# roymor1/OptimalStrategiesAgainstGenerativeAttacks

Measured on AMD Instinct MI355X. Metric: GIM episodes/sec (64x64x3, m=1 n=5 k=10), higher is better.
Workload: dtype f32

## Files before the change

### include/gim_hip.h

```cpp
#ifndef GIM_HIP_H
#define GIM_HIP_H

#include <stddef.h>
#include <stdint.h>

#ifdef __cplusplus
extern "C" {
#endif

#define GIM_OK 0
#define GIM_E_BADARG (-1)
#define GIM_E_LAUNCH (-2)

const char* gim_last_error(void);
int gim_version(void);

typedef struct {
    int32_t N, H, W, Cin, Cout, KH, ups;
    float pre_slope;
    int32_t pool, wfold, res_ups;
    int32_t tune_tile, tune_ksplit, tune_wgrad;
    int32_t out_zeroed;
    float post_slope;
    int32_t prec;
} gim_conv_shape;

int gim_conv2d_fold_weights(const float* w, float* f, int Cout, int Cin, int KH, void* stream);
typedef struct {
    const float* w;
    float* f;
    int32_t Cout, Cin, KH, reserved;
} gim_fold_job;
int gim_conv2d_fold_weights_batched(const gim_fold_job* jobs, const int32_t* tab, int n_blocks, void* stream);

int gim_conv2d_fwd(const float* x, const float* w, const float* bias, const float* sigma, const float* residual,
                   float* y, const gim_conv_shape* s, void* stream);

int gim_conv2d_dgrad(const float* dy, const float* w, const float* sigma, const float* mask_x, float* dx,
                     const gim_conv_shape* s, void* stream);

int gim_conv2d_dgrad_res(const float* dy, const float* w, const float* sigma, const float* mask_x, const float* res_half,
                         float res_scale, float* dx, const gim_conv_shape* s, void* stream);

int gim_conv2d_wgrad_slabs(const gim_conv_shape* s);
int gim_conv2d_wgrad(const float* dy, const float* x, float* slabs, float* bias_slabs, int n_slabs, const gim_conv_shape* s,
                     void* stream);

int gim_wgrad_finish(const float* slabs, const float* bias_slabs, int n_slabs, const float* w, const float* sigma,
                     const float* u, const float* v, float* dw, float* db, float* scratch, int Cout, int Cin, int KH,
                     int fold, float* acc_dw, float* acc_db, void* stream);

int gim_spectral_sigma(const float* w, float* u, float* v, float* sigma, float* u_out, float* v_out, float* scratch,
                       int Cout, int Cin, int KH, int training, void* stream);

typedef struct {
    const float* w;
    float* u;
    float* v;
    int64_t off_sigma, off_u, off_v, off_scratch;
    int32_t Cout, Cin, KH, reserved;
} gim_sn_job;
int gim_spectral_sigma_batched(const gim_sn_job* jobs, int n_jobs, const int32_t* tab_cols, int n_col_blocks,
                               const int32_t* tab_rows, int n_row_blocks, float* out_base, int training, void* stream);

int gim_conv2d_transpose_weights(const float* w, float* wt, int Cout, int Cin, int KF, void* stream);
int gim_conv2d_dgrad_t(const float* dy, const float* wt, const float* sigma, const float* mask_x, float* dx,
                       const gim_conv_shape* shape, void* stream);

int gim_conv2d_xfold_weights(const float* w, float* wx, int Cout, int Cin, int KH, int J, void* stream);
int gim_conv2d_dgrad_xfold(const float* dy, const float* wx, const float* sigma, const float* mask_x, float* dx,
                           const gim_conv_shape* shape, int J, void* stream);

int gim_pad_image(const float* x, float* xp, int N, int H, int W, int C, int pad, float slope, void* stream);
int gim_conv2d_pack_rows_weights(const float* w, float* wp, int Cout, int Cin, int KH, void* stream);
int gim_conv2d_fwd_rows(const float* xp, const float* wp, const float* bias, const float* sigma, const float* residual,
                        float* y, const gim_conv_shape* shape, void* stream);
int gim_conv2d_wgrad_rows_acc(const float* dy, const float* xp, float* acc, float* bias_acc, const gim_conv_shape* shape, void* stream);

int gim_conv2d_pack_subpixel_weights(const float* wf, float* wm, int Cout, int Cin, int KH, void* stream);
int gim_depth_to_space2(const float* y4, const float* bias, float* y, int N, int Hs, int Ws, int C, float post_slope, void* stream);

int gim_conv_launch_plan(const gim_conv_shape* shape, int kind, int32_t* out);

int gim_conv2d_wgrad_acc(const float* dy, const float* x, float* acc, float* bias_acc, const gim_conv_shape* shape, void* stream);

typedef struct {
    const float* src;
    const float* bias_src;
    const float* w;
    const float* sigma;
    const float* u;
    const float* v;
    float* tmp;
    float* partial;
    float* grad_w;
    float* grad_b;
    int32_t Cout, Cin, K, fold;
    int32_t n_chunks, exclusive;
} gim_wgrad_job;
int gim_wgrad_finish_batched(const gim_wgrad_job* jobs, int n_jobs, const int32_t* tab, int n_blocks, const int32_t* tab_sn,
                             int n_blocks_sn, void* stream);

int gim_colsum(const float* x, float* out, float* scratch, int64_t rows, int C, void* stream);

int gim_colsum_acc(const float* x, float* out, float* scratch, int64_t rows, int C, void* stream);
int gim_colsum2(const float* a, const float* b, float* out_a, float* out_b, int rows, int C, int accumulate, void* stream);

int gim_norm_fwd(const float* x, const float* scale, const float* shift, const float* residual, float* y, float* stats,
                 int N, int HW, int C, int mode, float eps, void* stream);
int gim_norm_fwd_act(const float* x, const float* scale, const float* shift, const float* residual, float* y, float* stats,
                     int N, int HW, int C, int mode, float eps, float post_slope, void* stream);
int gim_norm_bwd(const float* dy, const float* x, const float* scale, const float* stats, float* dx, float* dscale_nc,
                 float* dshift_nc, int N, int HW, int C, int mode, void* stream);

int gim_avgpool2_fwd(const float* x, float* y, int N, int H, int W, int C, void* stream);
int gim_avgpool2_fwd_act(const float* x, float* y, int N, int H, int W, int C, float in_slope, void* stream);
int gim_add_n(const float* a, const float* b, const float* c, const float* d, float* out, int64_t n, void* stream);
int gim_add_avgpool2_bwd(const float* g, const float* dy_pooled, float* out, int N, int H, int W, int C, void* stream);
int gim_avgpool2_bwd(const float* dy, float* dx, int N, int H, int W, int C, void* stream);
int gim_upsample2x_bwd(const float* dy_up, const float* mask_x, float slope, float* dx, int N, int H, int W, int C, void* stream);

int gim_maxpool_lrelu_fwd(const float* x, float* y, int32_t* idx, int N, int HW, int C, float slope, void* stream);
int gim_maxpool_lrelu_bwd(const float* dy, const float* y, const int32_t* idx, float* dx, int N, int HW, int C, float slope, void* stream);

int gim_attn_prob_fwd(const float* f, const float* g, float* P, int batch, int T, int K, void* stream);

int gim_bgemm(const float* A, const float* B, float* C, int batch, int M, int N, int K,
              int64_t sAb, int64_t sAi, int64_t sAk, int64_t sBb, int64_t sBk, int64_t sBj, void* stream);

typedef struct {
    const float* A;
    const float* B;
    float* C;
    const float* bias;
    int32_t M, N, K, ldc;
    int64_t sAi, sAk, sBk, sBj;
    int32_t flags, reserved;
} gim_gemm_job;
int gim_bgemm_grouped(const gim_gemm_job* jobs, const int32_t* tiles, int n_tiles, void* stream);
int gim_colsum_grouped(const gim_gemm_job* jobs, const int32_t* tiles, int n_tiles, void* stream);

int gim_softmax_dim1_fwd(const float* s, float* p, int B, int R, int Ccols, void* stream);
int gim_softmax_dim1_bwd(const float* dp, const float* p, float* ds, int B, int R, int Ccols, void* stream);

int gim_scale_add_fwd(const float* a, const float* x, const float* gamma, float* y, int64_t n, void* stream);
int gim_scale_add_fwd_act(const float* a, const float* x, const float* gamma, float* y, int64_t n, float post_slope, void* stream);
// ... 73 lines not shown
```

### optimalstrategiesagainstgenerativeattacks_amd/_lib.py

```python
import ctypes
import os
from ctypes import POINTER, c_float, c_int, c_int32, c_int64, c_void_p

_HERE = os.path.dirname(os.path.abspath(__file__))
LIB_PATH = os.environ.get("GIM_LIB_PATH") or os.path.join(_HERE, "csrc", "libgim_hip.so")


class GimConvShape(ctypes.Structure):
    _fields_ = [("N", c_int32), ("H", c_int32), ("W", c_int32), ("Cin", c_int32), ("Cout", c_int32),
                ("KH", c_int32), ("ups", c_int32), ("pre_slope", c_float),
                ("pool", c_int32), ("wfold", c_int32), ("res_ups", c_int32),
                ("tune_tile", c_int32), ("tune_ksplit", c_int32), ("tune_wgrad", c_int32),
                ("out_zeroed", c_int32), ("post_slope", c_float), ("prec", c_int32)]


class GimInferConv(ctypes.Structure):
    _fields_ = [("N", c_int32), ("H", c_int32), ("W", c_int32), ("Cin", c_int32), ("Cout", c_int32),
                ("KH", c_int32), ("stride", c_int32)]


P = c_void_p
SP = POINTER(GimConvShape)


class GimFoldJob(ctypes.Structure):
    _fields_ = [("w", P), ("f", P), ("Cout", c_int32), ("Cin", c_int32), ("KH", c_int32), ("reserved", c_int32)]


class GimSnJob(ctypes.Structure):
    _fields_ = [("w", P), ("u", P), ("v", P), ("off_sigma", c_int64), ("off_u", c_int64), ("off_v", c_int64), ("off_scratch", c_int64),
                ("Cout", c_int32), ("Cin", c_int32), ("KH", c_int32), ("reserved", c_int32)]


class GimWgradJob(ctypes.Structure):
    _fields_ = [("src", P), ("bias_src", P), ("w", P), ("sigma", P), ("u", P), ("v", P), ("tmp", P), ("partial", P),
                ("grad_w", P), ("grad_b", P), ("Cout", c_int32), ("Cin", c_int32), ("K", c_int32), ("fold", c_int32),
                ("n_chunks", c_int32), ("exclusive", c_int32)]


class GimGemmJob(ctypes.Structure):
    _fields_ = [("A", P), ("B", P), ("C", P), ("bias", P), ("M", c_int32), ("N", c_int32), ("K", c_int32), ("ldc", c_int32),
                ("sAi", c_int64), ("sAk", c_int64), ("sBk", c_int64), ("sBj", c_int64), ("flags", c_int32), ("reserved", c_int32)]


SIGNATURES = {
    "gim_conv2d_fwd": [P, P, P, P, P, P, SP, P],
    "gim_conv2d_dgrad": [P, P, P, P, P, SP, P],
    "gim_conv2d_dgrad_res": [P, P, P, P, P, c_float, P, SP, P],
    "gim_conv2d_wgrad_slabs": [SP],
    "gim_conv2d_wgrad": [P, P, P, P, c_int, SP, P],
    "gim_wgrad_finish": [P, P, c_int, P, P, P, P, P, P, P, c_int, c_int, c_int, c_int, P, P, P],
    "gim_conv2d_fold_weights": [P, P, c_int, c_int, c_int, P],
    "gim_conv2d_fold_weights_batched": [P, P, c_int, P],
    "gim_spectral_sigma": [P, P, P, P, P, P, P, c_int, c_int, c_int, c_int, P],
    "gim_spectral_sigma_batched": [P, c_int, P, c_int, P, c_int, P, c_int, P],
    "gim_colsum": [P, P, P, c_int64, c_int, P],
    "gim_norm_fwd": [P, P, P, P, P, P, c_int, c_int, c_int, c_int, c_float, P],
    "gim_norm_fwd_act": [P, P, P, P, P, P, c_int, c_int, c_int, c_int, c_float, c_float, P],
    "gim_norm_bwd": [P, P, P, P, P, P, P, c_int, c_int, c_int, c_int, P],
    "gim_avgpool2_fwd": [P, P, c_int, c_int, c_int, c_int, P],
    "gim_avgpool2_fwd_act": [P, P, c_int, c_int, c_int, c_int, c_float, P],
    "gim_add_n": [P, P, P, P, P, c_int64, P],
    "gim_add_avgpool2_bwd": [P, P, P, c_int, c_int, c_int, c_int, P],
    "gim_avgpool2_bwd": [P, P, c_int, c_int, c_int, c_int, P],
    "gim_upsample2x_bwd": [P, P, c_float, P, c_int, c_int, c_int, c_int, P],
    "gim_maxpool_lrelu_fwd": [P, P, P, c_int, c_int, c_int, c_float, P],
    "gim_maxpool_lrelu_bwd": [P, P, P, P, c_int, c_int, c_int, c_float, P],
    "gim_bgemm": [P, P, P, c_int, c_int, c_int, c_int, c_int64, c_int64, c_int64, c_int64, c_int64, c_int64, P],
    "gim_attn_prob_fwd": [P, P, P, c_int, c_int, c_int, P],
    "gim_softmax_dim1_fwd": [P, P, c_int, c_int, c_int, P],
    "gim_softmax_dim1_bwd": [P, P, P, c_int, c_int, c_int, P],
    "gim_bgemm_grouped": [P, P, c_int, P],
    "gim_colsum_grouped": [P, P, c_int, P],
    "gim_scale_add_fwd": [P, P, P, P, c_int64, P],
    "gim_scale_add_fwd_act": [P, P, P, P, c_int64, c_float, P],
    "gim_scale_add_bwd": [P, P, P, P, P, P, c_int64, P],
    "gim_tanh_fwd": [P, P, c_int64, P],
    "gim_tanh_bwd": [P, P, P, c_int64, P],
    "gim_nchw_to_nhwc": [P, P, c_int, c_int, c_int, P],
    "gim_nhwc_to_nchw": [P, P, c_int, c_int, c_int, P],
    "gim_set_stats_fwd": [P, P, P, c_int, c_int, c_int, c_int64, c_int64, P],
    "gim_set_stats_bwd": [P, P, P, P, c_int, c_int, c_int, c_int64, c_int64, P],
    "gim_bce_logits_fwd": [P, P, c_float, c_int, P],
    "gim_bce_logits_bwd": [P, P, P, c_float, c_int, P],
    "gim_sum_dim1": [P, P, c_int, c_int, c_int, c_float, P],
    "gim_repeat_dim1": [P, P, c_int, c_int, c_int, c_float, P],
    "gim_noise_combine": [P, P, P, c_int, c_int, c_int, c_int, P],
    "gim_concat2": [P, P, P, c_int64, c_int, c_int, c_int, c_int, P],
    "gim_slice_channels": [P, P, c_int64, c_int, c_int, P],
    "gim_conv2d_wgrad_acc": [P, P, P, P, SP, P],
    "gim_wgrad_finish_batched": [P, c_int, P, c_int, P, c_int, P],
    "gim_colsum_acc": [P, P, P, c_int64, c_int, P],
    "gim_colsum2": [P, P, P, P, c_int, c_int, c_int, P],
    "gim_conv_launch_plan": [SP, c_int, P],
    "gim_conv2d_transpose_weights": [P, P, c_int, c_int, c_int, P],
    "gim_conv2d_dgrad_t": [P, P, P, P, P, SP, P],
    "gim_conv2d_xfold_weights": [P, P, c_int, c_int, c_int, c_int, P],
    "gim_conv2d_dgrad_xfold": [P, P, P, P, P, SP, c_int, P],
    "gim_episode_gather": [P, P, P, P, c_int, c_int, c_int, c_int, P],
    "gim_resize_bilinear_u8": [P, c_int64, c_int, c_int, c_int, c_int, P, c_int, c_int, P, P, c_int, P, P, c_int, P],
    "gim_maxpool_gather": [P, P, P, P, c_int, c_int, c_int, c_float, P],
    "gim_softmax_dim1_bwd_dp": [P, P, P, P, c_int, c_int, c_int, P],
    "gim_set_stats_bwd_bwd": [P, P, P, P, P, P, c_int, c_int, c_int, c_int64, c_int64, P],
    "gim_lrelu_mask_mul": [P, P, c_float, P, c_int64, P],
    "gim_sqsum_rows_fwd": [P, P, c_int, c_int64, P],
    "gim_sqsum_rows_bwd": [P, P, P, c_int, c_int64, P],
    "gim_img_att_mix_fwd": [P, P, P, P, P, P, P, P, c_int64, c_int, P],
    "gim_img_att_mix_bwd": [P, P, P, P, P, P, P, P, P, P, P, P, P, P, c_int64, c_int, P],
    "gim_adam_step": [P, P, P, P, c_int64, P, P, c_int, c_float, c_float, c_float, c_float, P, P],
    "gim_adam_step_scaled": [P, P, P, P, c_int64, P, P, c_int, c_float, c_float, c_float, c_float, P, P, P],
    "gim_spin": [c_int, P],
    "gim_pad_image": [P, P, c_int, c_int, c_int, c_int, c_int, c_float, P],
    "gim_conv2d_pack_rows_weights": [P, P, c_int, c_int, c_int, P],
    "gim_conv2d_pack_subpixel_weights": [P, P, c_int, c_int, c_int, P],
    "gim_depth_to_space2": [P, P, P, c_int, c_int, c_int, c_int, c_float, P],
    "gim_conv2d_fwd_rows": [P, P, P, P, P, P, SP, P],
    "gim_conv2d_wgrad_rows_acc": [P, P, P, P, SP, P],
    "gim_conv2d_infer": [P, P, P, P, P, POINTER(GimInferConv), P],
    "gim_maxpool2_act": [P, P, c_int, c_int, c_int, c_int, c_int, P],
    "gim_channel_affine": [P, P, P, P, c_int64, c_int, P],
    "gim_se_tail": [P, P, P, P, P, P, P, c_int, c_int, c_int, c_int, c_int, P],
    "gim_pair_score": [P, P, P, c_int, c_int, P],
    "gim_l2norm_rows": [P, P, c_int, c_int, P],
    "gim_absdiff": [P, P, P, c_int64, P],
    "gim_version": [],
}

_lib = None


def load():
    global _lib
    if _lib is not None:
        return _lib
    if not os.path.exists(LIB_PATH):
        raise RuntimeError(
            "libgim_hip.so not found at %s: the HIP extension is not built "
            "(run __graft_entry__.build()); there is no CPU fallback" % LIB_PATH)
# ... 16 lines not shown
```

### optimalstrategiesagainstgenerativeattacks_amd/csrc/spectral.hip

```cpp
#include "common.h"

#define SN_R 8

__global__ __launch_bounds__(256) void sn_colpart_kernel(const float* __restrict__ w, const float* __restrict__ u,
                                                         float* __restrict__ part, int Cout, int K, int rows_per) {
    const int p = blockIdx.x * 256 + threadIdx.x;
    const int r = blockIdx.y;
    const int c0 = r * rows_per, c1 = min(Cout, c0 + rows_per);
    if (p >= K) return;
    float acc = 0.f;
    for (int co = c0; co < c1; ++co) acc += w[(long long)co * K + p] * u[co];
    part[(long long)r * K + p] = acc;
}

__global__ __launch_bounds__(256) void sn_vnorm_kernel(const float* __restrict__ part, int R, float* __restrict__ v,
                                                       float* __restrict__ v_phys, float* __restrict__ v_out, int K, int Cin,
                                                       int T, int training) {
    __shared__ float red[4];
    if (training) {
        float ss = 0.f;
        for (int p = threadIdx.x; p < K; p += 256) {
            float a = 0.f;
            for (int r = 0; r < R; ++r) a += part[(long long)r * K + p];
            v_phys[p] = a;
// ... 137 lines not shown
        const int kh = (int)(rr % K);
        const int co = (int)(rr / K);
        float g = 0.f;
#pragma unroll
        for (int dh = 0; dh < 2; ++dh)
#pragma unroll
            for (int dwd = 0; dwd < 2; ++dwd) {
                const int a = kh + dh, b = kw + dwd;
                if (fold == 1) g += src[(((long long)co * KF + a) * KF + b) * Cin + ci];
                else g += src[(((long long)ci * KF + (K - a)) * KF + (K - b)) * Cout + co];
            }
        if (fold == 1) g *= 0.25f;
        dw[i] = g;
        if (w) dot += g * w[i];
    }
    if (partial) {
        dot = block_sum_256(dot, red);
        if (threadIdx.x == 0) partial[blockIdx.x] = dot;
    }
}

__global__ __launch_bounds__(256) void wgrad_sn_apply_kernel(const float* __restrict__ g, float* __restrict__ dw, int accumulate,
                                                             const float* __restrict__ partial, int n_part,
                                                             const float* __restrict__ sigma, const float* __restrict__ u,
                                                             const float* __restrict__ v, long long n, int Cin, int T) {
    __shared__ float red[4];
    float d = 0.f;
    for (int i = threadIdx.x; i < n_part; i += 256) d += partial[i];
    d = block_sum_256(d, red);
    const float s = sigma[0];
    const float inv = 1.0f / s;
    const float coef = d * inv * inv;
    const int K = Cin * T;
    for (long long i = (long long)blockIdx.x * 256 + threadIdx.x; i < n; i += (long long)gridDim.x * 256) {
        const int co = (int)(i / K);
        const int p = (int)(i - (long long)co * K);
        const int tap = p / Cin, ci = p - tap * Cin;
        const float val = g[i] * inv - coef * u[co] * v[ci * T + tap];
        dw[i] = accumulate ? dw[i] + val : val;
    }
}

extern "C" int gim_wgrad_finish(const float* slabs, const float* bias_slabs, int n_slabs, const float* w, const float* sigma,
                                const float* u, const float* v, float* dw, float* db, float* scratch, int Cout, int Cin, int KH,
                                int fold, float* acc_dw, float* acc_db, void* stream) {
    GIM_CHECK_ARG(slabs && dw && n_slabs > 0, "wgrad_finish: bad args");
    GIM_CHECK_ARG((!db && !acc_db) || bias_slabs, "wgrad_finish: db needs bias_slabs");
    GIM_CHECK_ARG(!sigma || (w && u && v && scratch), "wgrad_finish: spectral form needs w, u, v, scratch");
    GIM_CHECK_ARG(fold >= 0 && fold <= 2 && (!fold || scratch), "wgrad_finish: bad fold / missing scratch");
    hipStream_t st = (hipStream_t)stream;
    const int T = KH * KH;
    const long long n = (long long)Cout * Cin * T;
    int blocks = (int)((n + 1023) / 1024);
    if (blocks > WF_BLOCKS) blocks = WF_BLOCKS;
    if (blocks < 1) blocks = 1;
    int sblocks = (int)((n + 63) / 64);
    if (sblocks > WF_BLOCKS) sblocks = WF_BLOCKS;
    float* bias_out = acc_db ? acc_db : db;
    const int bias_acc = acc_db ? 1 : 0;
    const bool direct = !sigma && !fold && acc_dw;
    if (fold == 0) {
        hipLaunchKernelGGL(wgrad_sum_kernel, dim3(sblocks), dim3(256), 0, st, slabs, n_slabs, n, sigma ? w : nullptr,
                           direct ? acc_dw : dw, sigma ? scratch : nullptr, bias_slabs, bias_out, Cout, direct ? 1 : 0, bias_acc);
        blocks = sblocks;
    } else {
        const long long nf = (long long)Cout * Cin * (KH + 1) * (KH + 1);
        float* fsum = scratch + WF_BLOCKS;
        int fb = (int)((nf + 63) / 64);
        if (fb > WF_BLOCKS) fb = WF_BLOCKS;
        hipLaunchKernelGGL(wgrad_sum_kernel, dim3(fb), dim3(256), 0, st, slabs, n_slabs, nf, (const float*)nullptr, fsum,
                           (float*)nullptr, bias_slabs, bias_out, Cout, 0, bias_acc);
        hipLaunchKernelGGL(wgrad_unfold_kernel, dim3(blocks), dim3(256), 0, st, fsum, sigma ? w : nullptr, dw,
                           sigma ? scratch : nullptr, Cout, Cin, KH, fold);
    }
    if (sigma) {
        hipLaunchKernelGGL(wgrad_sn_apply_kernel, dim3(blocks), dim3(256), 0, st, dw, acc_dw ? acc_dw : dw, acc_dw ? 1 : 0, scratch,
                           blocks, sigma, u, v, n, Cin, T);
    } else if (acc_dw && !direct) {
        GIM_CHECK_ARG(false, "wgrad_finish: acc_dw without sigma is only supported for fold == 0");
    }
    return gim_check_launch("gim_wgrad_finish");
}

__global__ __launch_bounds__(256) void snb_colpart_kernel(const gim_sn_job* __restrict__ jobs, const int4* __restrict__ tab,
                                                          float* __restrict__ out_base) {
    const int4 e = tab[blockIdx.x];
    const gim_sn_job jb = jobs[e.x];
    const int K = jb.Cin * jb.KH * jb.KH;
    const int p = e.y * 256 + threadIdx.x;
    if (p >= K) return;
    const int c0 = e.z * e.w, c1 = min(jb.Cout, c0 + e.w);
    float acc = 0.f;
    for (int co = c0; co < c1; ++co) acc += jb.w[(long long)co * K + p] * jb.u[co];
    (out_base + jb.off_scratch)[(long long)e.z * K + p] = acc;
}

__global__ __launch_bounds__(1024) void snb_vnorm_kernel(const gim_sn_job* __restrict__ jobs, float* __restrict__ out_base, int training) {
    __shared__ float red[16];
    const gim_sn_job jb = jobs[blockIdx.x];
    const int T = jb.KH * jb.KH, K = jb.Cin * T;
    const int R = min(SN_R, (jb.Cout + 63) / 64);
    float* part = out_base + jb.off_scratch;
    float* v_phys = part + (long long)SN_R * K;
    float* v_out = out_base + jb.off_v;
    if (training) {
        float ss = 0.f;
        for (int p = threadIdx.x; p < K; p += 1024) {
            float a = 0.f;
            for (int r = 0; r < R; ++r) a += part[(long long)r * K + p];
            v_phys[p] = a;
            ss += a * a;
        }
        ss = wave_sum(ss);
        if ((threadIdx.x & 63) == 0) red[threadIdx.x >> 6] = ss;
        __syncthreads();
        float tot = 0.f;
#pragma unroll
        for (int i = 0; i < 16; ++i) tot += red[i];
        const float inv = 1.0f / fmaxf(sqrtf(tot), 1e-12f);
        for (int p = threadIdx.x; p < K; p += 1024) {
            const float val = v_phys[p] * inv;
            const int tap = p / jb.Cin, ci = p - tap * jb.Cin;
            const int q = ci * T + tap;
            v_phys[p] = val;
            jb.v[q] = val;
            v_out[q] = val;
        }
    } else {
        for (int q = threadIdx.x; q < K; q += 1024) {
            const int ci = q / T, tap = q - ci * T;
            const float val = jb.v[q];
            v_phys[tap * jb.Cin + ci] = val;
            v_out[q] = val;
        }
    }
}

__global__ __launch_bounds__(256) void snb_rowdot_kernel(const gim_sn_job* __restrict__ jobs, const int2* __restrict__ tab,
                                                         float* __restrict__ out_base) {
    const int2 e = tab[blockIdx.x];
    const gim_sn_job jb = jobs[e.x];
    const int K = jb.Cin * jb.KH * jb.KH;
    const int co = e.y * 4 + (threadIdx.x >> 6);
    const int lane = threadIdx.x & 63;
    if (co >= jb.Cout) return;
    const float* v_phys = out_base + jb.off_scratch + (long long)SN_R * K;
    float* tvec = out_base + jb.off_scratch + (long long)(SN_R + 1) * K;
    const float* row = jb.w + (long long)co * K;
    float acc = 0.f;
    for (int p = lane; p < K; p += 64) acc += row[p] * v_phys[p];
    acc = wave_sum(acc);
    if (lane == 0) tvec[co] = acc;
}

__global__ __launch_bounds__(256) void snb_final_kernel(const gim_sn_job* __restrict__ jobs, float* __restrict__ out_base, int training) {
    __shared__ float red[4];
    const gim_sn_job jb = jobs[blockIdx.x];
    const int K = jb.Cin * jb.KH * jb.KH;
    const float* tvec = out_base + jb.off_scratch + (long long)(SN_R + 1) * K;
    float* u_out = out_base + jb.off_u;
    float inv = 0.f;
    if (training) {
        float ss = 0.f;
        for (int c = threadIdx.x; c < jb.Cout; c += 256) ss += tvec[c] * tvec[c];
        inv = 1.0f / fmaxf(sqrtf(block_sum_256(ss, red)), 1e-12f);
    }
    float dot = 0.f;
    for (int c = threadIdx.x; c < jb.Cout; c += 256) {
        float uv;
        if (training) {
            uv = tvec[c] * inv;
            jb.u[c] = uv;
        } else {
            uv = jb.u[c];
        }
        u_out[c] = uv;
        dot += uv * tvec[c];
    }
    dot = block_sum_256(dot, red);
    if (threadIdx.x == 0) (out_base + jb.off_sigma)[0] = dot;
}

extern "C" int gim_spectral_sigma_batched(const gim_sn_job* jobs, int n_jobs, const int32_t* tab_cols, int n_col_blocks,
                                          const int32_t* tab_rows, int n_row_blocks, float* out_base, int training, void* stream) {
    GIM_CHECK_ARG(jobs && n_jobs > 0 && tab_cols && tab_rows && out_base && n_col_blocks > 0 && n_row_blocks > 0,
                  "spectral_sigma_batched: bad args");
    hipStream_t st = (hipStream_t)stream;
    if (training)
        hipLaunchKernelGGL(snb_colpart_kernel, dim3(n_col_blocks), dim3(256), 0, st, jobs, reinterpret_cast<const int4*>(tab_cols), out_base);
    hipLaunchKernelGGL(snb_vnorm_kernel, dim3(n_jobs), dim3(1024), 0, st, jobs, out_base, training);
    hipLaunchKernelGGL(snb_rowdot_kernel, dim3(n_row_blocks), dim3(256), 0, st, jobs, reinterpret_cast<const int2*>(tab_rows), out_base);
    hipLaunchKernelGGL(snb_final_kernel, dim3(n_jobs), dim3(256), 0, st, jobs, out_base, training);
    return gim_check_launch("gim_spectral_sigma_batched");
}

#define WGQ_CHUNK 4096

__device__ __forceinline__ float wgq_load(const gim_wgrad_job& jb, unsigned i) {
    if (jb.fold == 0) return jb.src[i];
    const unsigned K = jb.K, KF = K + 1, Cin = jb.Cin, Cout = jb.Cout;
    const unsigned r1 = i / Cin, ci = i - r1 * Cin;
    const unsigned r2 = r1 / K, kw = r1 - r2 * K;
    if (jb.fold == 3)
        return jb.src[r2 * ((K * Cin + 15u) & ~15u) + kw * Cin + ci];
    const unsigned co = r2 / K, kh = r2 - co * K;
    float g = 0.f;
#pragma unroll
    for (unsigned dh = 0; dh < 2; ++dh)
#pragma unroll
        for (unsigned dwd = 0; dwd < 2; ++dwd) {
            const unsigned a = kh + dh, b = kw + dwd;
            if (jb.fold == 1) g += jb.src[((co * KF + a) * KF + b) * Cin + ci];
            else g += jb.src[((ci * KF + (K - a)) * KF + (K - b)) * Cout + co];
        }
    return jb.fold == 1 ? 0.25f * g : g;
}

__device__ __forceinline__ bool wgq_aligned16(const void* a, const void* b, const void* c) {
    return (((uintptr_t)a | (uintptr_t)b | (uintptr_t)c) & 15) == 0;
}

__global__ __launch_bounds__(256) void wgq_reduce_kernel(const gim_wgrad_job* __restrict__ jobs, const int2* __restrict__ tab) {
    __shared__ float red[4];
    const int2 e = tab[blockIdx.x];
    const gim_wgrad_job jb = jobs[e.x];
    const unsigned n = (unsigned)jb.Cout * jb.K * jb.K * jb.Cin;
    const unsigned i0 = (unsigned)e.y * WGQ_CHUNK;
    const unsigned cnt = min((unsigned)WGQ_CHUNK, n - i0);
    const bool sn = jb.sigma != nullptr;
    float dot = 0.f;
    if (sn && jb.fold == 2 && (jb.Cout & 63) == 0 && (jb.Cin & 63) == 0) {
        __shared__ float tile[64][65];
        const unsigned K = jb.K, KF = K + 1, T = K * K, Cin = jb.Cin, Cout = jb.Cout, tiles_ci = Cin >> 6;
        const unsigned tap = (unsigned)e.y % T, r = (unsigned)e.y / T;
        const unsigned ci0 = (r % tiles_ci) << 6, co0 = (r / tiles_ci) << 6;
        const unsigned kh = tap / K, kw = tap - kh * K;
        const unsigned lane = threadIdx.x & 63, wv = threadIdx.x >> 6;
#pragma unroll 4
        for (unsigned j = 0; j < 16; ++j) {
            const unsigned ci = ci0 + wv + 4 * j;
            const float* base = jb.src + (((size_t)ci * KF + (K - kh)) * KF + (K - kw)) * Cout + co0 + lane;
            tile[wv + 4 * j][lane] = (base[0] + base[-(long)Cout]) + (base[-(long)(KF * Cout)] + base[-(long)((KF + 1) * Cout)]);
        }
        __syncthreads();
#pragma unroll 4
        for (unsigned j = 0; j < 16; ++j) {
            const unsigned co = co0 + wv + 4 * j;
            const float g = tile[lane][wv + 4 * j];
            const unsigned i = ((co * K + kh) * K + kw) * Cin + ci0 + lane;
            jb.tmp[i] = g;
            dot += g * jb.w[i];
        }
    } else if (sn && jb.fold == 0 && (n & 3) == 0 && wgq_aligned16(jb.src, jb.w, jb.w)) {
        for (unsigned t = threadIdx.x * 4; t < cnt; t += 1024) {
            const float4 g = *reinterpret_cast<const float4*>(jb.src + i0 + t);
            const float4 w = *reinterpret_cast<const float4*>(jb.w + i0 + t);
            dot += g.x * w.x + g.y * w.y + g.z * w.z + g.w * w.w;
        }
    } else if (!sn && jb.fold == 0 && jb.exclusive && (n & 3) == 0 && wgq_aligned16(jb.src, jb.grad_w, jb.grad_w)) {
        for (unsigned t = threadIdx.x * 4; t < cnt; t += 1024) {
            const float4 g = *reinterpret_cast<const float4*>(jb.src + i0 + t);
            float4* dst = reinterpret_cast<float4*>(jb.grad_w + i0 + t);
            float4 o = *dst;
            o.x += g.x; o.y += g.y; o.z += g.z; o.w += g.w;
            *dst = o;
        }
    } else {
#pragma unroll 4
        for (unsigned t = threadIdx.x; t < cnt; t += 256) {
            const unsigned i = i0 + t;
            const float g = wgq_load(jb, i);
            if (sn) {
                if (jb.fold) jb.tmp[i] = g;
                dot += g * jb.w[i];
            } else {
// ... 74 lines not shown
```

### optimalstrategiesagainstgenerativeattacks_amd/model_blocks.py

```python
import collections
import math

import torch
import torch.nn as nn

from . import _lib
from . import ops

LRELU = 0.2


def _kaiming_uniform_like_torch(weight, bias, fan_in):
    nn.init.kaiming_uniform_(weight, a=math.sqrt(5))
    if bias is not None:
        bound = 1.0 / math.sqrt(fan_in) if fan_in > 0 else 0.0
        nn.init.uniform_(bias, -bound, bound)


class GimLinear(nn.Module):

    def __init__(self, in_features, out_features):
        super().__init__()
        self.in_features, self.out_features = in_features, out_features
        self.weight = nn.Parameter(torch.empty(out_features, in_features))
# ... 31 lines not shown
                slope = LRELU
            else:
                x = layer(x, pre_slope=slope)
                slope = 1.0
        return x


class SNConv2d(nn.Module):

    def __init__(self, in_channels, out_channels, kernel_size, padding=0):
        super().__init__()
        assert padding == (kernel_size - 1) // 2, "only 'same' stride-1 convolutions are on the GIM hot path"
        self.in_channels, self.out_channels, self.kernel_size = in_channels, out_channels, kernel_size
        w = torch.empty(out_channels, in_channels, kernel_size, kernel_size)
        b = torch.empty(out_channels)
        _kaiming_uniform_like_torch(w, b, in_channels * kernel_size * kernel_size)
        u = nn.functional.normalize(w.new_empty(out_channels).normal_(0, 1), dim=0, eps=1e-12)
        v = nn.functional.normalize(w.new_empty(in_channels * kernel_size * kernel_size).normal_(0, 1), dim=0, eps=1e-12)
        self.bias = nn.Parameter(b)
        self.weight_orig = nn.Parameter(w.contiguous(memory_format=torch.channels_last))
        self.register_buffer("weight_u", u)
        self.register_buffer("weight_v", v)

        self._sn_queue = collections.deque()
        self._wants_fold = False
        self._fold_slot = (kernel_size + 1, "fold")

    def fold_is_stale(self):
        return ops._WT_CACHE.is_stale(self.weight_orig, self._fold_slot)

    def folded(self):
        self._wants_fold = True
        return ops._WT_CACHE.get(self.weight_orig, self._fold_slot, lambda: ops._folded(
            ops.weight_phys(self.weight_orig), self.out_channels, self.in_channels, self.kernel_size))

    def forward(self, x, res=None, ups=0, pre_slope=1.0, pool=False, res_ups=False, post_slope=1.0, x_act=False, fork_pool_slope=None):
        guard = None
        if self._sn_queue:
            sigma, u_s, v_s, guard = self._sn_queue.popleft()
        else:
            sigma, u_s, v_s = ops.spectral_sigma(self.weight_orig, self.weight_u, self.weight_v, self.training)
        if fork_pool_slope is not None:
            assert res is None and not ups and not pool and not res_ups
            return ops.conv2d_forkpool(x, self.weight_orig, self.bias, sigma, u_s, v_s, pre_slope, guard, post_slope, x_act, fork_pool_slope)
        wf = self.folded() if (pool or (ups and self.kernel_size > 1)) else None
        if post_slope != 1.0:
            return ops.conv2d_post_act(x, self.weight_orig, self.bias, res, sigma, u_s, v_s, ups, pre_slope, pool, res_ups, wf, guard, post_slope, x_act)
        return ops.conv2d(x, self.weight_orig, self.bias, res, sigma, u_s, v_s, ups, pre_slope, pool, res_ups, wf, guard, x_act)

    def extra_repr(self):
        return "%d, %d, kernel_size=%d (spectral norm)" % (self.in_channels, self.out_channels, self.kernel_size)


class SNPlan:

    def __init__(self, convs):
        self.convs = [c for c in convs if isinstance(c, SNConv2d)]
        self._gen = 0
        self._bufs = {}
        self._tables = ops._TableCache("SNPlan", 1)
        self._fold_tables = ops._TableCache("SNPlan folds", None, skip_in_capture=True)

    def stale(self, gen):
        return self._gen - gen > 2

    def _build(self):
        jobs = (_lib.GimSnJob * len(self.convs))()
        cols, rows, views = [], [], []
        off = 0

        def take(n):
            nonlocal off
            o = off
            off += (n + 3) // 4 * 4
            return o
        for j, c in enumerate(self.convs):
            Cout, Cin, KH = c.out_channels, c.in_channels, c.kernel_size
            K = Cin * KH * KH
            if not c.weight_orig.permute(0, 2, 3, 1).is_contiguous():
                raise RuntimeError("SNPlan: weight_orig must be stored channels-last")
            o_s, o_u, o_v, o_scr = take(1), take(Cout), take(K), take(10 * K + Cout)
            jobs[j] = (c.weight_orig.data_ptr(), c.weight_u.data_ptr(), c.weight_v.data_ptr(), o_s, o_u, o_v, o_scr, Cout, Cin, KH, 0)
            R = min(8, (Cout + 63) // 64)
            rows_per = (Cout + R - 1) // R
            for xb in range((K + 255) // 256):
                for r in range(R):
                    cols.append((j, xb, r, rows_per))
            for rb in range((Cout + 3) // 4):
                rows.append((j, rb))
            views.append((o_s, o_u, Cout, o_v, K))
        return ops._DeviceTable(jobs, cols, rows, extra=(len(jobs), len(cols), len(rows), off, views))

    @torch.no_grad()
    def run(self, rounds, training):
        if not self.convs:
            return
        w0 = self.convs[0].weight_orig
        if not (w0.is_cuda and w0.dtype == torch.float32):
            raise RuntimeError("weights must be CUDA float32 (got %s on %s): the GIM engine has no CPU path" % (w0.dtype, w0.device))
        tab = self._tables.get(tuple(t.data_ptr() for c in self.convs for t in (c.weight_orig, c.weight_u, c.weight_v)), self._build)
        (d_jobs, d_cols, d_rows), (n_jobs, n_cols, n_rows, total, views) = tab.ptrs, tab.extra
        raw = ops._stream()
        tab.use_on_current_stream(raw)
        for c in self.convs:
            c._sn_queue.clear()
        gen = self._gen
        self._gen += 1
        for r in range(rounds):
            out = self._bufs.get((gen & 1, r))
            if out is None or out.numel() != total or out.device != w0.device:
                out = self._bufs[(gen & 1, r)] = torch.empty(total, device=w0.device, dtype=torch.float32)
            _lib.check(_lib.load().gim_spectral_sigma_batched(d_jobs, n_jobs, d_cols, n_cols, d_rows, n_rows, out.data_ptr(), 1 if training else 0, raw),
                       "spectral_sigma_batched")
            for c, (o_s, o_u, Cout, o_v, K) in zip(self.convs, views):
                c._sn_queue.append((out[o_s:o_s + 1], out[o_u:o_u + Cout], out[o_v:o_v + K], (self, gen)))
        self._fold_stale(raw)

    def _fold_stale(self, raw):
        todo = [c for c in self.convs if c._wants_fold and c.fold_is_stale()]
        if len(todo) < 2:
            return

        def build():
            jobs = (_lib.GimFoldJob * len(todo))()
            bufs, chunks = [], []
            for j, c in enumerate(todo):
                KF = c.kernel_size + 1
                n = c.out_channels * KF * KF * c.in_channels
                if n >= 1 << 31:
                    raise RuntimeError("folded weights of more than 2^31 elements (gim_conv2d_fold_weights_batched indexes with 32 bits)")
                bufs.append(torch.empty(n, device=c.weight_orig.device, dtype=torch.float32))
                jobs[j] = (c.weight_orig.data_ptr(), bufs[j].data_ptr(), c.out_channels, c.in_channels, c.kernel_size, 0)
                chunks += [(j, ch) for ch in range((n + 65535) // 65536)]
            return ops._DeviceTable(jobs, chunks, extra=(len(chunks), bufs))
        tab = self._fold_tables.get(tuple(c.weight_orig.data_ptr() for c in todo), build)
        if tab is None:
            return
        tab.use_on_current_stream(raw)
        _lib.check(_lib.load().gim_conv2d_fold_weights_batched(tab.ptrs[0], tab.ptrs[1], tab.extra[0], raw), "fold_weights_batched")
        for c, f in zip(todo, tab.extra[1]):
            ops._WT_CACHE.install(c.weight_orig, c._fold_slot, f)


def sn_convs(*modules):
    return [m for mod in modules for m in mod.modules() if isinstance(m, SNConv2d)]


class GimInstanceNorm2d(nn.Module):

    def __init__(self, num_features, eps=1e-5):
        super().__init__()
        self.num_features, self.eps = num_features, eps
        self.weight = nn.Parameter(torch.ones(num_features))
        self.bias = nn.Parameter(torch.zeros(num_features))

    def forward(self, x, post_slope=1.0):
        return ops.instance_norm(x, self.weight, self.bias, self.eps, post_slope)


def custom_std(x):
    D = x.shape[-1]
    return ops.mean_std_cat(x)[:, D:]


class ResBlockDown(nn.Module):

    def __init__(self, in_channel, out_channel, conv_size=3, padding_size=1):
        super().__init__()
        self.conv_l1 = SNConv2d(in_channel, out_channel, 1)
        self.conv_r1 = SNConv2d(in_channel, out_channel, conv_size, padding=padding_size)
        self.conv_r2 = SNConv2d(out_channel, out_channel, conv_size, padding=padding_size)

    def forward(self, x):
        return self.forward_act(x)[0]

    def forward_act(self, x, x_act=False, post_slope=1.0):
        out, act, pooled = self.conv_r1(x, pre_slope=LRELU, post_slope=LRELU, x_act=x_act, fork_pool_slope=LRELU if x_act else 1.0)
        left = self.conv_l1(pooled)
        if post_slope != 1.0 and ops.act_storage():
            return self.conv_r2(out, res=left, pre_slope=LRELU, pool=True, x_act=act, post_slope=post_slope)
        return self.conv_r2(out, res=left, pre_slope=LRELU, pool=True, x_act=act), False


class SelfAttention(nn.Module):

    def __init__(self, in_channel):
        super().__init__()
        self.conv_f = SNConv2d(in_channel, in_channel // 8, 1)
        self.conv_g = SNConv2d(in_channel, in_channel // 8, 1)
        self.conv_h = SNConv2d(in_channel, in_channel, 1)
        self.gamma = nn.Parameter(torch.zeros(1))

    def forward(self, x, post_slope=1.0):
        N, H, W, C = x.shape
        xf, xg, xh, xr = ops.fork(x, 4)
# ... 108 lines not shown
```

Measured before the change: 435.5.

## Fuse batched spectral-norm power iteration into two kernels with last-block tickets

Replaces the four-kernel batched spectral-norm power iteration with two kernels. Per-job atomic ticket counters let the last arriving block do the v-normalisation and the final sigma/u reduction, so the separate vnorm and final launches are removed. It also widens column blocks to 1024 with float4 loads and unrolls the row dot products, with rows-per-wave chosen by K. This cuts launch count and serialisation gaps at the cost of atomic counters, relaxed-publish memory ordering that must be correct, and less parallelism in the tail reductions.

```diff
diff --git a/include/gim_hip.h b/include/gim_hip.h
--- a/include/gim_hip.h
+++ b/include/gim_hip.h
@@ -61,7 +61,8 @@
     int32_t Cout, Cin, KH, reserved;
 } gim_sn_job;
 int gim_spectral_sigma_batched(const gim_sn_job* jobs, int n_jobs, const int32_t* tab_cols, int n_col_blocks,
-                               const int32_t* tab_rows, int n_row_blocks, float* out_base, int training, void* stream);
+                               const int32_t* tab_rows, int n_row_blocks, float* out_base, int32_t* tickets, int training,
+                               void* stream);
 
 int gim_conv2d_transpose_weights(const float* w, float* wt, int Cout, int Cin, int KF, void* stream);
 int gim_conv2d_dgrad_t(const float* dy, const float* wt, const float* sigma, const float* mask_x, float* dx,
diff --git a/optimalstrategiesagainstgenerativeattacks_amd/_lib.py b/optimalstrategiesagainstgenerativeattacks_amd/_lib.py
--- a/optimalstrategiesagainstgenerativeattacks_amd/_lib.py
+++ b/optimalstrategiesagainstgenerativeattacks_amd/_lib.py
@@ -53,7 +53,7 @@
     "gim_conv2d_fold_weights": [P, P, c_int, c_int, c_int, P],
     "gim_conv2d_fold_weights_batched": [P, P, c_int, P],
     "gim_spectral_sigma": [P, P, P, P, P, P, P, c_int, c_int, c_int, c_int, P],
-    "gim_spectral_sigma_batched": [P, c_int, P, c_int, P, c_int, P, c_int, P],
+    "gim_spectral_sigma_batched": [P, c_int, P, c_int, P, c_int, P, P, c_int, P],
     "gim_colsum": [P, P, P, c_int64, c_int, P],
     "gim_norm_fwd": [P, P, P, P, P, P, c_int, c_int, c_int, c_int, c_float, P],
     "gim_norm_fwd_act": [P, P, P, P, P, P, c_int, c_int, c_int, c_int, c_float, c_float, P],
diff --git a/optimalstrategiesagainstgenerativeattacks_amd/csrc/spectral.hip b/optimalstrategiesagainstgenerativeattacks_amd/csrc/spectral.hip
--- a/optimalstrategiesagainstgenerativeattacks_amd/csrc/spectral.hip
+++ b/optimalstrategiesagainstgenerativeattacks_amd/csrc/spectral.hip
@@ -243,82 +243,181 @@
     return gim_check_launch("gim_wgrad_finish");
 }
 
-__global__ __launch_bounds__(256) void snb_colpart_kernel(const gim_sn_job* __restrict__ jobs, const int4* __restrict__ tab,
-                                                          float* __restrict__ out_base) {
+#define SNB_COLS 1024
+
+__device__ __forceinline__ void snb_publish(float* dst, float v) {
+    __hip_atomic_store(dst, v, __ATOMIC_RELAXED, __HIP_MEMORY_SCOPE_AGENT);
+}
+__device__ __forceinline__ void snb_publish4(float* dst, float4 v) {
+    unsigned long long* d = reinterpret_cast<unsigned long long*>(dst);
+    __hip_atomic_store(d, ((unsigned long long)__float_as_uint(v.y) << 32) | __float_as_uint(v.x), __ATOMIC_RELAXED, __HIP_MEMORY_SCOPE_AGENT);
+    __hip_atomic_store(d + 1, ((unsigned long long)__float_as_uint(v.w) << 32) | __float_as_uint(v.z), __ATOMIC_RELAXED, __HIP_MEMORY_SCOPE_AGENT);
+}
+
+__device__ __forceinline__ bool snb_last_arriver(int* cnt, int total, float* flag) {
+    asm volatile("s_waitcnt vmcnt(0)" ::: "memory");
+    __syncthreads();
+    if (threadIdx.x == 0) {
+        const int ticket = __hip_atomic_fetch_add(cnt, 1, __ATOMIC_RELAXED, __HIP_MEMORY_SCOPE_AGENT);
+        const bool last = ticket == total - 1;
+        if (last) {
+            __hip_atomic_store(cnt, 0, __ATOMIC_RELAXED, __HIP_MEMORY_SCOPE_AGENT);
+            __builtin_amdgcn_fence(__ATOMIC_ACQUIRE, "agent");
+            asm volatile("s_waitcnt vmcnt(0)" ::: "memory");
+        }
+        *flag = last ? 1.f : 0.f;
+    }
+    __syncthreads();
+    return *flag != 0.f;
+}
+
+__global__ __launch_bounds__(256) void snb_colpass_kernel(const gim_sn_job* __restrict__ jobs, const int4* __restrict__ tab,
+                                                          float* __restrict__ out_base, int* __restrict__ tickets, int training) {
+    __shared__ float red[17];
+    const int4 e = tab[blockIdx.x];
+    const gim_sn_job jb = jobs[e.x];
+    const int T = jb.KH * jb.KH, K = jb.Cin * T;
+    const int R = min(SN_R, (jb.Cout + 63) / 64);
+    const int rows_per = (jb.Cout + R - 1) / R;
+    float* part = out_base + jb.off_scratch;
+    float* v_phys = part + (long long)SN_R * K;
+    float* v_out = out_base + jb.off_v;
+    const int t = threadIdx.x, p0 = e.y * SNB_COLS;
+    if (!training) {
+        if (e.z == 0)
+            for (int p = p0 + t; p < min(K, p0 + SNB_COLS); p += 256) {
+                const int tap = p / jb.Cin, ci = p - tap * jb.Cin;
+                const int q = ci * T + tap;
+                const float val = jb.v[q];
+                v_phys[p] = val;
+                v_out[q] = val;
+            }
+        return;
+    }
+    const int c0 = e.z * rows_per, c1 = min(jb.Cout, c0 + rows_per);
+    if ((K & 3) == 0 && ((uintptr_t)jb.w & 15) == 0) {
+        const int p = p0 + 4 * t;
+        if (p < K) {
+            float4 acc = make_float4(0.f, 0.f, 0.f, 0.f);
+            const float* col = jb.w + (long long)c0 * K + p;
+            int co = c0;
+            for (; co + 8 <= c1; co += 8, col += 8LL * K) {
+                float4 x[8];
+#pragma unroll
+                for (int i = 0; i < 8; ++i) x[i] = *reinterpret_cast<const float4*>(col + (long long)i * K);
+#pragma unroll
+                for (int i = 0; i < 8; ++i) {
+                    const float uc = jb.u[co + i];
+                    acc.x += x[i].x * uc; acc.y += x[i].y * uc; acc.z += x[i].z * uc; acc.w += x[i].w * uc;
+                }
+            }
+            for (; co < c1; ++co, col += K) {
+                const float4 x = *reinterpret_cast<const float4*>(col);
+                const float uc = jb.u[co];
+                acc.x += x.x * uc; acc.y += x.y * uc; acc.z += x.z * uc; acc.w += x.w * uc;
+            }
+            snb_publish4(part + (long long)e.z * K + p, acc);
+        }
+    } else {
+        float acc[4] = {0.f, 0.f, 0.f, 0.f};
+        int pc[4];
+#pragma unroll
+        for (int j = 0; j < 4; ++j) pc[j] = min(p0 + t + 256 * j, K - 1);
+        const float* row = jb.w + (long long)c0 * K;
+        int co = c0;
+        for (; co + 4 <= c1; co += 4, row += 4LL * K) {
+            float x[4][4];
+#pragma unroll
+            for (int i = 0; i < 4; ++i)
+#pragma unroll
+                for (int j = 0; j < 4; ++j) x[i][j] = row[(long long)i * K + pc[j]];
+#pragma unroll
+            for (int i = 0; i < 4; ++i) {
+                const float uc = jb.u[co + i];
+#pragma unroll
+                for (int j = 0; j < 4; ++j) acc[j] += x[i][j] * uc;
+            }
+        }
+        for (; co < c1; ++co, row += K) {
+            const float uc = jb.u[co];
+#pragma unroll
+            for (int j = 0; j < 4; ++j) acc[j] += row[pc[j]] * uc;
+        }
+#pragma unroll
+        for (int j = 0; j < 4; ++j) {
+            const int p = p0 + t + 256 * j;
+            if (p < K) snb_publish(part + (long long)e.z * K + p, acc[j]);
+        }
+    }
+    if (!snb_last_arriver(tickets + 2 * e.x, e.w, &red[16])) return;
+
+    float ss[4] = {0.f, 0.f, 0.f, 0.f};
+    for (int pb = t; pb < K; pb += 1024) {
+#pragma unroll
+        for (int j = 0; j < 4; ++j) {
+            const int p = pb + 256 * j;
+            if (p < K) {
+                float pr[SN_R];
+#pragma unroll
+                for (int r = 0; r < SN_R; ++r) pr[r] = part[(long long)min(r, R - 1) * K + p];
+                float a = 0.f;
+#pragma unroll
+                for (int r = 0; r < SN_R; ++r) a = r < R ? a + pr[r] : a;
+                v_phys[p] = a;
+                ss[j] += a * a;
+            }
+        }
+    }
+#pragma unroll
+    for (int j = 0; j < 4; ++j) {
+        const float s = wave_sum(ss[j]);
+        if ((t & 63) == 0) red[4 * j + (t >> 6)] = s;
+    }
+    __syncthreads();
+    float tot = 0.f;
+#pragma unroll
+    for (int i = 0; i < 16; ++i) tot += red[i];
+    const float inv = 1.0f / fmaxf(sqrtf(tot), 1e-12f);
+    for (int p = t; p < K; p += 256) {
+        const float val = v_phys[p] * inv;
+        const int tap = p / jb.Cin, ci = p - tap * jb.Cin;
+        const int q = ci * T + tap;
+        v_phys[p] = val;
+        jb.v[q] = val;
+        v_out[q] = val;
+    }
+}
+
+__global__ __launch_bounds__(256) void snb_rowpass_kernel(const gim_sn_job* __restrict__ jobs, const int4* __restrict__ tab,
+                                                          float* __restrict__ out_base, int* __restrict__ tickets, int training) {
+    __shared__ float red[5];
     const int4 e = tab[blockIdx.x];
     const gim_sn_job jb = jobs[e.x];
     const int K = jb.Cin * jb.KH * jb.KH;
-    const int p = e.y * 256 + threadIdx.x;
-    if (p >= K) return;
-    const int c0 = e.z * e.w, c1 = min(jb.Cout, c0 + e.w);
-    float acc = 0.f;
-    for (int co = c0; co < c1; ++co) acc += jb.w[(long long)co * K + p] * jb.u[co];
-    (out_base + jb.off_scratch)[(long long)e.z * K + p] = acc;
-}
-
-__global__ __launch_bounds__(1024) void snb_vnorm_kernel(const gim_sn_job* __restrict__ jobs, float* __restrict__ out_base, int training) {
-    __shared__ float red[16];
-    const gim_sn_job jb = jobs[blockIdx.x];
-    const int T = jb.KH * jb.KH, K = jb.Cin * T;
-    const int R = min(SN_R, (jb.Cout + 63) / 64);
-    float* part = out_base + jb.off_scratch;
-    float* v_phys = part + (long long)SN_R * K;
-    float* v_out = out_base + jb.off_v;
-    if (training) {
-        float ss = 0.f;
-        for (int p = threadIdx.x; p < K; p += 1024) {
-            float a = 0.f;
-            for (int r = 0; r < R; ++r) a += part[(long long)r * K + p];
-            v_phys[p] = a;
-            ss += a * a;
-        }
-        ss = wave_sum(ss);
-        if ((threadIdx.x & 63) == 0) red[threadIdx.x >> 6] = ss;
-        __syncthreads();
-        float tot = 0.f;
-#pragma unroll
-        for (int i = 0; i < 16; ++i) tot += red[i];
-        const float inv = 1.0f / fmaxf(sqrtf(tot), 1e-12f);
-        for (int p = threadIdx.x; p < K; p += 1024) {
-            const float val = v_phys[p] * inv;
-            const int tap = p / jb.Cin, ci = p - tap * jb.Cin;
-            const int q = ci * T + tap;
-            v_phys[p] = val;
-            jb.v[q] = val;
-            v_out[q] = val;
-        }
-    } else {
-        for (int q = threadIdx.x; q < K; q += 1024) {
-            const int ci = q / T, tap = q - ci * T;
-            const float val = jb.v[q];
-            v_phys[tap * jb.Cin + ci] = val;
-            v_out[q] = val;
-        }
-    }
-}
-
-__global__ __launch_bounds__(256) void snb_rowdot_kernel(const gim_sn_job* __restrict__ jobs, const int2* __restrict__ tab,
-                                                         float* __restrict__ out_base) {
-    const int2 e = tab[blockIdx.x];
-    const gim_sn_job jb = jobs[e.x];
-    const int K = jb.Cin * jb.KH * jb.KH;
-    const int co = e.y * 4 + (threadIdx.x >> 6);
     const int lane = threadIdx.x & 63;
-    if (co >= jb.Cout) return;
     const float* v_phys = out_base + jb.off_scratch + (long long)SN_R * K;
     float* tvec = out_base + jb.off_scratch + (long long)(SN_R + 1) * K;
-    const float* row = jb.w + (long long)co * K;
-    float acc = 0.f;
-    for (int p = lane; p < K; p += 64) acc += row[p] * v_phys[p];
-    acc = wave_sum(acc);
-    if (lane == 0) tvec[co] = acc;
-}
-
-__global__ __launch_bounds__(256) void snb_final_kernel(const gim_sn_job* __restrict__ jobs, float* __restrict__ out_base, int training) {
-    __shared__ float red[4];
-    const gim_sn_job jb = jobs[blockIdx.x];
-    const int K = jb.Cin * jb.KH * jb.KH;
-    const float* tvec = out_base + jb.off_scratch + (long long)(SN_R + 1) * K;
+    const int row0 = (e.y * 4 + (threadIdx.x >> 6)) * e.w;
+    for (int co = row0; co < min(jb.Cout, row0 + e.w); ++co) {
+        const float* row = jb.w + (long long)co * K;
+        float acc = 0.f;
+        int p = lane;
+        for (; p + 7 * 64 < K; p += 8 * 64) {
+            float x[8], y[8];
+#pragma unroll
+            for (int i = 0; i < 8; ++i) {
+                x[i] = row[p + 64 * i];
+                y[i] = v_phys[p + 64 * i];
+            }
+#pragma unroll
+            for (int i = 0; i < 8; ++i) acc = __builtin_fmaf(x[i], y[i], acc);
+        }
+        for (; p < K; p += 64) acc = __builtin_fmaf(row[p], v_phys[p], acc);
+        acc = wave_sum(acc);
+        if (lane == 0) snb_publish(tvec + co, acc);
+    }
+    if (!snb_last_arriver(tickets + 2 * e.x + 1, e.z, &red[4])) return;
+
     float* u_out = out_base + jb.off_u;
     float inv = 0.f;
     if (training) {
@@ -343,15 +442,16 @@
 }
 
 extern "C" int gim_spectral_sigma_batched(const gim_sn_job* jobs, int n_jobs, const int32_t* tab_cols, int n_col_blocks,
-                                          const int32_t* tab_rows, int n_row_blocks, float* out_base, int training, void* stream) {
-    GIM_CHECK_ARG(jobs && n_jobs > 0 && tab_cols && tab_rows && out_base && n_col_blocks > 0 && n_row_blocks > 0,
+                                          const int32_t* tab_rows, int n_row_blocks, float* out_base, int32_t* tickets, int training,
+                                          void* stream) {
+    GIM_CHECK_ARG(jobs && n_jobs > 0 && tab_cols && tab_rows && out_base && tickets && n_col_blocks > 0 && n_row_blocks > 0,
                   "spectral_sigma_batched: bad args");
+    GIM_CHECK_ARG(!((uintptr_t)out_base & 15), "spectral_sigma_batched: out_base on a 16-byte boundary");
     hipStream_t st = (hipStream_t)stream;
-    if (training)
-        hipLaunchKernelGGL(snb_colpart_kernel, dim3(n_col_blocks), dim3(256), 0, st, jobs, reinterpret_cast<const int4*>(tab_cols), out_base);
-    hipLaunchKernelGGL(snb_vnorm_kernel, dim3(n_jobs), dim3(1024), 0, st, jobs, out_base, training);
-    hipLaunchKernelGGL(snb_rowdot_kernel, dim3(n_row_blocks), dim3(256), 0, st, jobs, reinterpret_cast<const int2*>(tab_rows), out_base);
-    hipLaunchKernelGGL(snb_final_kernel, dim3(n_jobs), dim3(256), 0, st, jobs, out_base, training);
+    hipLaunchKernelGGL(snb_colpass_kernel, dim3(n_col_blocks), dim3(256), 0, st, jobs, reinterpret_cast<const int4*>(tab_cols), out_base,
+                       tickets, training);
+    hipLaunchKernelGGL(snb_rowpass_kernel, dim3(n_row_blocks), dim3(256), 0, st, jobs, reinterpret_cast<const int4*>(tab_rows), out_base,
+                       tickets, training);
     return gim_check_launch("gim_spectral_sigma_batched");
 }
 
diff --git a/optimalstrategiesagainstgenerativeattacks_amd/model_blocks.py b/optimalstrategiesagainstgenerativeattacks_amd/model_blocks.py
--- a/optimalstrategiesagainstgenerativeattacks_amd/model_blocks.py
+++ b/optimalstrategiesagainstgenerativeattacks_amd/model_blocks.py
@@ -137,14 +137,14 @@
             o_s, o_u, o_v, o_scr = take(1), take(Cout), take(K), take(10 * K + Cout)
             jobs[j] = (c.weight_orig.data_ptr(), c.weight_u.data_ptr(), c.weight_v.data_ptr(), o_s, o_u, o_v, o_scr, Cout, Cin, KH, 0)
             R = min(8, (Cout + 63) // 64)
-            rows_per = (Cout + R - 1) // R
-            for xb in range((K + 255) // 256):
-                for r in range(R):
-                    cols.append((j, xb, r, rows_per))
-            for rb in range((Cout + 3) // 4):
-                rows.append((j, rb))
+            n_cb = (K + 1023) // 1024
+            cols += [(j, xb, r, n_cb * R) for xb in range(n_cb) for r in range(R)]
+            rpw = 1 if K > 512 else 2 if K > 128 else 4
+            n_rb = (Cout + 4 * rpw - 1) // (4 * rpw)
+            rows += [(j, rb, n_rb, rpw) for rb in range(n_rb)]
             views.append((o_s, o_u, Cout, o_v, K))
-        return ops._DeviceTable(jobs, cols, rows, extra=(len(jobs), len(cols), len(rows), off, views))
+        tickets = [(0, 0)] * len(jobs)
+        return ops._DeviceTable(jobs, cols, rows, tickets, extra=(len(jobs), len(cols), len(rows), off, views))
 
     @torch.no_grad()
     def run(self, rounds, training):
@@ -154,7 +154,7 @@
         if not (w0.is_cuda and w0.dtype == torch.float32):
             raise RuntimeError("weights must be CUDA float32 (got %s on %s): the GIM engine has no CPU path" % (w0.dtype, w0.device))
         tab = self._tables.get(tuple(t.data_ptr() for c in self.convs for t in (c.weight_orig, c.weight_u, c.weight_v)), self._build)
-        (d_jobs, d_cols, d_rows), (n_jobs, n_cols, n_rows, total, views) = tab.ptrs, tab.extra
+        (d_jobs, d_cols, d_rows, d_tickets), (n_jobs, n_cols, n_rows, total, views) = tab.ptrs, tab.extra
         raw = ops._stream()
         tab.use_on_current_stream(raw)
         for c in self.convs:
@@ -165,7 +165,8 @@
             out = self._bufs.get((gen & 1, r))
             if out is None or out.numel() != total or out.device != w0.device:
                 out = self._bufs[(gen & 1, r)] = torch.empty(total, device=w0.device, dtype=torch.float32)
-            _lib.check(_lib.load().gim_spectral_sigma_batched(d_jobs, n_jobs, d_cols, n_cols, d_rows, n_rows, out.data_ptr(), 1 if training else 0, raw),
+            _lib.check(_lib.load().gim_spectral_sigma_batched(d_jobs, n_jobs, d_cols, n_cols, d_rows, n_rows, out.data_ptr(), d_tickets,
+                                                              1 if training else 0, raw),
                        "spectral_sigma_batched")
             for c, (o_s, o_u, Cout, o_v, K) in zip(self.convs, views):
                 c._sn_queue.append((out[o_s:o_s + 1], out[o_u:o_u + Cout], out[o_v:o_v + K], (self, gen)))
```

Measured after the change: 436.3 (median of 6 runs). No clear change (+0.2%).
